# armlabstanford/Touch-GS

Measured on AMD Instinct MI355X. Metric: train iters/s (whole-job views/s) + render Mpix/s, 1M Gaussians @ 1080p, higher is better.
Workload: dtype f32; 1 GPU; configs[2]: 1M Gaussians, 1080p, full Touch-GS train loop (RGB L1/SSIM + tactile depth/uncertainty loss), one view per rank per iter; gaussians=1000000, width=1920, height=1080, sh_degree=3, views=8, tiles=8160, longest_tile_list_any_view=792, max_list_hint=1022, parallelism=dp1, layout=morton (model.spatial_sort(): same scene, rows permuted), depth_loss_type=DEPTH_UNCERTAINTY_WEIGHTED_LOSS

## Files before the change

### touch_gs_amd/csrc/imgloss.hip

```cpp
#include <math.h>
#include <stdlib.h>
#include "tgs_common.h"

namespace {

constexpr int WIN = 11, HALO = 5;
struct Win { float g[WIN]; };
#ifdef TGS_SSIM_SGPR_WINDOW
#define WK(k) win.g[k]
#else
__device__ constexpr float WGT[WIN] = {0x1.0d956cp-10f, 0x1.f1fe02p-8f, 0x1.26eb18p-5f, 0x1.bff0fep-4f, 0x1.b43c4p-3f,
                                       0x1.10656p-2f, 0x1.b43c4p-3f, 0x1.bff0fep-4f, 0x1.26eb18p-5f, 0x1.f1fe02p-8f,
                                       0x1.0d956cp-10f};
#define WK(k) WGT[k]
#endif

#ifndef TGS_SSIM_DMA
#define TGS_SSIM_DMA 0
#endif
constexpr int SW = 64;
constexpr int NTH = 3 * SW;
constexpr int RB = WIN;
__host__ __device__ constexpr int seg_rows(int nblk) { return RB * nblk - 2 * HALO; }

template <int CH>
struct RowBlock {
  static constexpr int ROWF = (SW + 2 * HALO) * CH;
  static constexpr int NIT = (RB * ROWF + NTH - 1) / NTH;
  template <int B = 8>
  static __device__ __forceinline__ void stage(const float* __restrict__ src, float* __restrict__ lds,
                                               int W, int H, int x0, int r0, int tid) {
#pragma unroll 1
    for (int it0 = 0; it0 < NIT; it0 += B) {
      float v[B];
#pragma unroll
      for (int u = 0; u < B; u++) {
        const int i = tid + NTH * (it0 + u);
        const int j = i / ROWF, e = i - j * ROWF;
        const int gy = r0 + j, gxf = (x0 - HALO) * CH + e;
        v[u] = 0.f;
        if (i < RB * ROWF && gy >= 0 && gy < H && gxf >= 0 && gxf < W * CH) v[u] = src[(size_t)gy * W * CH + gxf];
      }
#pragma unroll
      for (int u = 0; u < B; u++) {
        const int i = tid + NTH * (it0 + u);
        if (i < RB * ROWF) lds[i] = v[u];
      }
    }
  }
  static constexpr int PADF = (RB * ROWF + TGS_WAVE - 1) / TGS_WAVE * TGS_WAVE;
  static constexpr int NDMA = PADF / TGS_WAVE;
  static __device__ __forceinline__ void dma(__amdgpu_buffer_rsrc_t rsrc, float* __restrict__ lds, int W, int H, int x0, int r0, int tid) {
    typedef __attribute__((address_space(3))) float lds_float;
    const int wave = __builtin_amdgcn_readfirstlane(tid >> 6), lane = tid & 63;
    constexpr int NW = NTH / TGS_WAVE;
    const int gx0 = (x0 - HALO) * CH, WC = W * CH;
#pragma unroll
    for (int u = 0; u * NW < NDMA; u++) {
      const int chunk = u * NW + wave;
      if (chunk < NDMA) {
        const int i = chunk * TGS_WAVE + lane;
        const int j = i / ROWF, e = i - j * ROWF;
        const int gy = r0 + j, gxf = gx0 + e;
        const bool in = i < RB * ROWF && (unsigned)gy < (unsigned)H && (unsigned)gxf < (unsigned)WC;
        const unsigned off = in ? (unsigned)(gy * WC + gxf) * 4u : 0xffffffffu;
        __builtin_amdgcn_raw_ptr_buffer_load_lds(rsrc, (lds_float*)(lds + chunk * TGS_WAVE), 4, off, 0, 0, 0);
      }
    }
  }
  static __device__ __forceinline__ void stage2(const float* __restrict__ src_a, const float* __restrict__ src_b,
                                                float* __restrict__ lds_a, float* __restrict__ lds_b,
                                                int W, int H, int x0, int r0, int tid) {
#ifndef TGS_SSIM_FWD_B
#define TGS_SSIM_FWD_B 13
#endif
    constexpr int B = TGS_SSIM_FWD_B;
#pragma unroll 1
    for (int it0 = 0; it0 < NIT; it0 += B) {
      float va[B], vb[B];
#pragma unroll
      for (int u = 0; u < B; u++) {
        const int i = tid + NTH * (it0 + u);
        const int j = i / ROWF, e = i - j * ROWF;
        const int gy = r0 + j, gxf = (x0 - HALO) * CH + e;
        va[u] = 0.f; vb[u] = 0.f;
        if (it0 + u < NIT && i < RB * ROWF && gy >= 0 && gy < H && gxf >= 0 && gxf < W * CH) {
          const size_t o = (size_t)gy * W * CH + gxf;
          va[u] = src_a[o]; vb[u] = src_b[o];
        }
      }
#pragma unroll
      for (int u = 0; u < B; u++) {
        const int i = tid + NTH * (it0 + u);
        if (it0 + u < NIT && i < RB * ROWF) { lds_a[i] = va[u]; lds_b[i] = vb[u]; }
      }
    }
  }
};

__global__ __launch_bounds__(NTH) __attribute__((amdgpu_waves_per_eu(4, 8))) void k_ssim_fwd(int W, int H, Win win,
                                                  const float* __restrict__ img,
                                                  const float* __restrict__ gt,
                                                  float* __restrict__ adj ,
                                                  float* __restrict__ block_partials, int n_partials, int NBLK,
                                                  int y_lo, int y_hi, int c_lo, int c_hi) {
  const int SEG = seg_rows(NBLK);
  constexpr int ROWF = RowBlock<3>::ROWF;
#if TGS_SSIM_DMA & 1
  __shared__ float sa2[2][RowBlock<3>::PADF], sb2[2][RowBlock<3>::PADF];
  const __amdgpu_buffer_rsrc_t rs_a = __builtin_amdgcn_make_buffer_rsrc((void*)img, 0, (int)((size_t)W * H * 12), 0x00020000);
  const __amdgpu_buffer_rsrc_t rs_b = __builtin_amdgcn_make_buffer_rsrc((void*)gt, 0, (int)((size_t)W * H * 12), 0x00020000);
#else
  __shared__ float sa[RB * ROWF], sb[RB * ROWF];
#endif
  __shared__ float red[NTH / TGS_WAVE];
  const int tid = threadIdx.x;
  const int x0 = blockIdx.x * SW, ys = y_lo + blockIdx.y * SEG;
  const int gx = x0 + tid / 3, c = tid - (tid / 3) * 3;
  const int ye = min(ys + SEG, y_hi);
  float w[RB][5];
#pragma unroll
  for (int p = 0; p < RB; p++)
#pragma unroll
    for (int q = 0; q < 5; q++) w[p][q] = 0.f;
  float msum = 0.f;
#if TGS_SSIM_DMA & 1
  RowBlock<3>::dma(rs_a, sa2[0], W, H, x0, ys - HALO, tid);
  RowBlock<3>::dma(rs_b, sb2[0], W, H, x0, ys - HALO, tid);
#endif
  for (int blk = 0; blk < NBLK; blk++) {
    const int r0 = ys - HALO + blk * RB;
    if (r0 - HALO >= ye) break;
#if TGS_SSIM_DMA & 1
    asm volatile("s_waitcnt vmcnt(0)" ::: "memory");
    __syncthreads();
    if (blk + 1 < NBLK && r0 + RB - HALO < ye) {
      RowBlock<3>::dma(rs_a, sa2[(blk + 1) & 1], W, H, x0, r0 + RB, tid);
      RowBlock<3>::dma(rs_b, sb2[(blk + 1) & 1], W, H, x0, r0 + RB, tid);
    }
    const float* sa = sa2[blk & 1];
    const float* sb = sb2[blk & 1];
#else
    __syncthreads();
    {
      RowBlock<3>::stage2(img, gt, sa, sb, W, H, x0, r0, tid);
    }
    __syncthreads();
#endif
#pragma unroll
    for (int p = 0; p < RB; p++) {
      const float* ra = sa + p * ROWF + tid;
      const float* rb = sb + p * ROWF + tid;
      float m1 = 0.f, m2 = 0.f, e11 = 0.f, e22 = 0.f, e12 = 0.f;
#pragma unroll
      for (int k = 0; k < WIN; k++) {
        const float a = ra[3 * k], b = rb[3 * k];
        const float ga = WK(k) * a, gb = WK(k) * b;
        m1 += ga; m2 += gb;
        e11 = fmaf(ga, a, e11); e22 = fmaf(gb, b, e22); e12 = fmaf(ga, b, e12);
      }
      w[p][0] = m1; w[p][1] = m2; w[p][2] = e11; w[p][3] = e22; w[p][4] = e12;
      const int gy = r0 + p - HALO;
      if (gy >= ys && gy < ye) {
        float o[5] = {0.f, 0.f, 0.f, 0.f, 0.f};
#pragma unroll
        for (int k = 0; k < WIN; k++) {
#pragma unroll
          for (int q = 0; q < 5; q++) o[q] = fmaf(WK(k), w[(p + 1 + k) % RB][q], o[q]);
        }
        const float C1 = 0.01f * 0.01f, C2 = 0.03f * 0.03f;
        const float mu1 = o[0], mu2 = o[1];
        const float s11 = o[2] - mu1 * mu1, s22 = o[3] - mu2 * mu2, s12 = o[4] - mu1 * mu2;
        const float n1 = 2.f * mu1 * mu2 + C1, n2 = 2.f * s12 + C2;
        const float d1 = mu1 * mu1 + mu2 * mu2 + C1, d2 = s11 + s22 + C2;
        const float id1 = __builtin_amdgcn_rcpf(d1), id2 = __builtin_amdgcn_rcpf(d2);
        const float m = n1 * n2 * id1 * id2;
        if (gx < W) {
          if (gy >= c_lo && gy < c_hi) msum += m;
          if (adj) {
            const float dm_ds12 = 2.f * n1 * id1 * id2;
            const float dm_ds11 = -m * id2;
            const float dm_dmu1 = 2.f * mu2 * n2 * id1 * id2 - m * 2.f * mu1 * id1;
            float* o3 = adj + (((size_t)gy * W + gx) * 3 + c) * 3;
            o3[0] = dm_dmu1 - 2.f * mu1 * dm_ds11 - mu2 * dm_ds12;
            o3[1] = dm_ds11;
            o3[2] = dm_ds12;
          }
        }
      }
    }
  }
  const float tot = wave_sum(msum);
  if ((tid & 63) == 0) red[tid >> 6] = tot;
  __syncthreads();
  const int wg = blockIdx.y * gridDim.x + blockIdx.x, nwg = gridDim.x * gridDim.y;
  if (tid == 0) block_partials[wg] = red[0] + red[1] + red[2];
  for (int i = nwg + wg * NTH + tid; i < n_partials; i += nwg * NTH) block_partials[i] = 0.f;
}

__global__ __launch_bounds__(NTH) __attribute__((amdgpu_waves_per_eu(4, 8))) void k_ssim_bwd(int W, int H, Win win, float weight,
                                                  const float* __restrict__ img,
                                                  const float* __restrict__ gt,
                                                  const float* __restrict__ adj,
                                                  float* __restrict__ v_img, int NBLK, int y_lo, int y_hi) {
  const int SEG = seg_rows(NBLK);
  constexpr int ROWF = RowBlock<9>::ROWF;
#if TGS_SSIM_DMA & 2
  __shared__ float sadj2[2][RowBlock<9>::PADF];
  const __amdgpu_buffer_rsrc_t rs_j = __builtin_amdgcn_make_buffer_rsrc((void*)adj, 0, (int)((size_t)W * H * 36), 0x00020000);
#else
  __shared__ float sadj[RB * ROWF];
#endif
  const int tid = threadIdx.x;
  const int x0 = blockIdx.x * SW, ys = y_lo + blockIdx.y * SEG;
  const int gx = x0 + tid / 3;
  const int ye = min(ys + SEG, y_hi);
  float w[RB][3];
#pragma unroll
  for (int p = 0; p < RB; p++) { w[p][0] = 0.f; w[p][1] = 0.f; w[p][2] = 0.f; }
#if TGS_SSIM_DMA & 2
  RowBlock<9>::dma(rs_j, sadj2[0], W, H, x0, ys - HALO, tid);
#endif
  for (int blk = 0; blk < NBLK; blk++) {
    const int r0 = ys - HALO + blk * RB;
    if (r0 - HALO >= ye) break;
#if TGS_SSIM_DMA & 2
    asm volatile("s_waitcnt vmcnt(0)" ::: "memory");
    __syncthreads();
    if (blk + 1 < NBLK && r0 + RB - HALO < ye) RowBlock<9>::dma(rs_j, sadj2[(blk + 1) & 1], W, H, x0, r0 + RB, tid);
    const float* sadj = sadj2[blk & 1];
#else
    __syncthreads();
    {
#ifndef TGS_SSIM_BWD_B
#define TGS_SSIM_BWD_B 20
#endif
      RowBlock<9>::stage<TGS_SSIM_BWD_B>(adj, sadj, W, H, x0, r0, tid);
    }
    __syncthreads();
#endif
#pragma unroll
    for (int p = 0; p < RB; p++) {
      const float* r = sadj + p * ROWF + 3 * tid;
      float h0 = 0.f, h1 = 0.f, h2 = 0.f;
#pragma unroll
      for (int k = 0; k < WIN; k++) {
        h0 = fmaf(WK(k), r[9 * k], h0);
        h1 = fmaf(WK(k), r[9 * k + 1], h1);
        h2 = fmaf(WK(k), r[9 * k + 2], h2);
      }
      w[p][0] = h0; w[p][1] = h1; w[p][2] = h2;
      const int gy = r0 + p - HALO;
      if (gy >= ys && gy < ye) {
        float o0 = 0.f, o1 = 0.f, o2 = 0.f;
#pragma unroll
        for (int k = 0; k < WIN; k++) {
          o0 = fmaf(WK(k), w[(p + 1 + k) % RB][0], o0);
          o1 = fmaf(WK(k), w[(p + 1 + k) % RB][1], o1);
          o2 = fmaf(WK(k), w[(p + 1 + k) % RB][2], o2);
        }
        if (gx < W) {
          const size_t pidx = (size_t)gy * W * 3 + (size_t)x0 * 3 + tid;
          v_img[pidx] = weight * (o0 + 2.f * img[pidx] * o1 + gt[pidx] * o2);
        }
      }
    }
  }
}


constexpr int SWO = SW - 2 * HALO;
__host__ __device__ constexpr int fused_seg_rows(int nblk) { return RB * nblk - 4 * HALO; }

__global__ __launch_bounds__(NTH) __attribute__((amdgpu_waves_per_eu(3, 4))) void k_ssim_fused(
    int W, int H, float weight, const float* __restrict__ img, const float* __restrict__ gt,
    float* __restrict__ v_img, float* __restrict__ block_partials, int n_partials, int NBLK,
    int y_lo, int y_hi, int c_lo, int c_hi) {
  const int SEG = fused_seg_rows(NBLK);
  constexpr int ROWF = RowBlock<3>::ROWF;
  constexpr int ADJF = SW * 9;
  __shared__ float sa[RB * ROWF], sb[RB * ROWF];
  __shared__ float sadj[RB * ADJF];
  __shared__ float red[NTH / TGS_WAVE];
  const int tid = threadIdx.x;
  const int col = tid / 3, c = tid - col * 3;
  const int xa0 = blockIdx.x * SWO - HALO;
  const int gx = xa0 + col;
  const int ys = y_lo + blockIdx.y * SEG, ye = min(ys + SEG, y_hi);
  const bool own_col = col >= HALO && col < SW - HALO;
  const int cb = min(max(col - HALO, 0), SWO - 1);
  float w[RB][5], w2[RB][3];
#pragma unroll
  for (int p = 0; p < RB; p++) {
#pragma unroll
    for (int q = 0; q < 5; q++) w[p][q] = 0.f;
    w2[p][0] = 0.f; w2[p][1] = 0.f; w2[p][2] = 0.f;
  }
  float msum = 0.f;
  for (int blk = 0; blk < NBLK; blk++) {
    const int r0 = ys - 2 * HALO + blk * RB;
    if (r0 - 2 * HALO >= ye) break;
    __syncthreads();
    RowBlock<3>::stage2(img, gt, sa, sb, W, H, xa0, r0, tid);
    __syncthreads();
#pragma unroll
    for (int p = 0; p < RB; p++) {
      const float* ra = sa + p * ROWF + tid;
      const float* rb = sb + p * ROWF + tid;
      float m1 = 0.f, m2 = 0.f, e11 = 0.f, e22 = 0.f, e12 = 0.f;
#pragma unroll
      for (int k = 0; k < WIN; k++) {
        const float a = ra[3 * k], b = rb[3 * k];
        const float ga = WK(k) * a, gb = WK(k) * b;
        m1 += ga; m2 += gb;
        e11 = fmaf(ga, a, e11); e22 = fmaf(gb, b, e22); e12 = fmaf(ga, b, e12);
      }
      w[p][0] = m1; w[p][1] = m2; w[p][2] = e11; w[p][3] = e22; w[p][4] = e12;
      const int gy = r0 + p - HALO;
      float A = 0.f, B = 0.f, C = 0.f;
      if (gy >= ys - HALO && gy < ye + HALO && gy >= 0 && gy < H) {
        float o[5] = {0.f, 0.f, 0.f, 0.f, 0.f};
#pragma unroll
        for (int k = 0; k < WIN; k++) {
#pragma unroll
          for (int q = 0; q < 5; q++) o[q] = fmaf(WK(k), w[(p + 1 + k) % RB][q], o[q]);
        }
        const float C1 = 0.01f * 0.01f, C2 = 0.03f * 0.03f;
        const float mu1 = o[0], mu2 = o[1];
        const float s11 = o[2] - mu1 * mu1, s22 = o[3] - mu2 * mu2, s12 = o[4] - mu1 * mu2;
        const float n1 = 2.f * mu1 * mu2 + C1, n2 = 2.f * s12 + C2;
        const float d1 = mu1 * mu1 + mu2 * mu2 + C1, d2 = s11 + s22 + C2;
        const float id1 = __builtin_amdgcn_rcpf(d1), id2 = __builtin_amdgcn_rcpf(d2);
        const float m = n1 * n2 * id1 * id2;
        if (gx >= 0 && gx < W) {
          if (own_col && gy >= ys && gy < ye && gy >= c_lo && gy < c_hi) msum += m;
          const float dm_ds12 = 2.f * n1 * id1 * id2;
          const float dm_ds11 = -m * id2;
          const float dm_dmu1 = 2.f * mu2 * n2 * id1 * id2 - m * 2.f * mu1 * id1;
          A = dm_dmu1 - 2.f * mu1 * dm_ds11 - mu2 * dm_ds12;
          B = dm_ds11;
          C = dm_ds12;
        }
      }
      float* o3 = sadj + p * ADJF + tid * 3;
      o3[0] = A; o3[1] = B; o3[2] = C;
    }
    __syncthreads();
#pragma unroll
    for (int p = 0; p < RB; p++) {
      const float* r = sadj + p * ADJF + (cb * 3 + c) * 3;
      float h0 = 0.f, h1 = 0.f, h2 = 0.f;
#pragma unroll
      for (int k = 0; k < WIN; k++) {
        h0 = fmaf(WK(k), r[9 * k], h0);
        h1 = fmaf(WK(k), r[9 * k + 1], h1);
        h2 = fmaf(WK(k), r[9 * k + 2], h2);
      }
      w2[p][0] = h0; w2[p][1] = h1; w2[p][2] = h2;
      const int gy = r0 + p - 2 * HALO;
      if (gy >= ys && gy < ye) {
        float o0 = 0.f, o1 = 0.f, o2 = 0.f;
#pragma unroll
        for (int k = 0; k < WIN; k++) {
          o0 = fmaf(WK(k), w2[(p + 1 + k) % RB][0], o0);
          o1 = fmaf(WK(k), w2[(p + 1 + k) % RB][1], o1);
          o2 = fmaf(WK(k), w2[(p + 1 + k) % RB][2], o2);
        }
        if (own_col && gx < W) {
          const size_t pidx = ((size_t)gy * W + gx) * 3 + c;
          v_img[pidx] = weight * (o0 + 2.f * img[pidx] * o1 + gt[pidx] * o2);
        }
      }
    }
  }
  const float tot = wave_sum(msum);
  if ((tid & 63) == 0) red[tid >> 6] = tot;
  __syncthreads();
  const int wg = blockIdx.y * gridDim.x + blockIdx.x, nwg = gridDim.x * gridDim.y;
  if (tid == 0) block_partials[wg] = red[0] + red[1] + red[2];
  for (int i = nwg + wg * NTH + tid; i < n_partials; i += nwg * NTH) block_partials[i] = 0.f;
}

__global__ void k_ssim_zero_partials(float* __restrict__ block_partials, int n_partials) {
  const int i = blockIdx.x * blockDim.x + threadIdx.x;
  if (i < n_partials) block_partials[i] = 0.f;
}

}

static inline bool count_inside(int y0, int y1, int c0, int c1) { return c0 >= c1 || (c0 >= y0 && c1 <= y1); }

static int ssim_impl(int W, int H, const float* img, const float* gt, float weight,
                     float* block_partials, int n_partials, float* v_img, float* scratch,
                     int y0, int y1, int c0, int c1, void* stream) {
  TGS_CHECK_ARG(W > 0 && H > 0, "bad image size");
  TGS_CHECK_ARG(img && gt && block_partials, "null pointer");
  TGS_CHECK_ARG(!v_img || scratch, "gradient needs scratch");
  TGS_CHECK_ARG(0 <= y0 && y0 <= y1 && y1 <= H && y0 <= c0 && c0 <= c1 && c1 <= y1, "bad row range");
  Win win;
  double g[WIN], sum = 0.0;
  for (int i = 0; i < WIN; i++) { g[i] = exp(-(double)((i - HALO) * (i - HALO)) / (2.0 * 1.5 * 1.5)); sum += g[i]; }
  for (int i = 0; i < WIN; i++) win.g[i] = (float)(g[i] / sum);
  static const int env_nblk = [] { const char* e = getenv("TGS_SSIM_NBLK"); return e ? max(2, min(16, atoi(e))) : 0; }();
  static const int env_fused = [] { const char* e = getenv("TGS_SSIM_FUSED"); return e ? atoi(e) : 0; }();
  if (v_img && env_fused && y1 > y0 && count_inside(y0, y1, c0, c1)) {
    const int fx = (W + SWO - 1) / SWO;
    auto wgs = [&](int nb) { return (long long)fx * ((y1 - y0 + fused_seg_rows(nb) - 1) / fused_seg_rows(nb)); };
    int nblk = 7;
    while (nblk > 3 && wgs(nblk) < 600) nblk--;
    if (env_nblk) nblk = max(3, env_nblk);
    while (nblk < 16 && wgs(nblk) > n_partials) nblk++;
    TGS_CHECK_ARG(wgs(nblk) <= n_partials, "block_partials too small");
    const int SEGF = fused_seg_rows(nblk);
    hipLaunchKernelGGL(k_ssim_fused, dim3(fx, (y1 - y0 + SEGF - 1) / SEGF, 1), dim3(NTH), 0, (hipStream_t)stream, W, H, weight,
                       img, gt, v_img, block_partials, n_partials, nblk, y0, y1, c0, c1);
    TGS_CHECK_LAUNCH();
    return TGS_OK;
  }
  const int f0 = v_img ? max(0, y0 - HALO) : y0, f1 = v_img ? min(H, y1 + HALO) : y1;
  const int rows = f1 - f0;
  if (rows <= 0) {
    if (n_partials > 0) {
      hipLaunchKernelGGL(k_ssim_zero_partials, dim3((n_partials + 255) / 256), dim3(256), 0, (hipStream_t)stream, block_partials,
                         n_partials);
      TGS_CHECK_LAUNCH();
    }
    return TGS_OK;
  }
  const int sx = (W + SW - 1) / SW;
  int nblk = 4;
  while (nblk > 2 && (long long)sx * ((rows + seg_rows(nblk) - 1) / seg_rows(nblk)) < 3 * 256) nblk--;
  if (env_nblk) nblk = env_nblk;
  while (nblk < 16 && (long long)sx * ((rows + seg_rows(nblk) - 1) / seg_rows(nblk)) > n_partials) nblk++;
  TGS_CHECK_ARG((long long)sx * ((rows + seg_rows(nblk) - 1) / seg_rows(nblk)) <= n_partials, "block_partials too small");
  const int SEG = seg_rows(nblk);
  const dim3 block(NTH);
  hipStream_t s = (hipStream_t)stream;
  hipLaunchKernelGGL(k_ssim_fwd, dim3(sx, (rows + SEG - 1) / SEG, 1), block, 0, s, W, H, win, img, gt,
                     v_img ? scratch : nullptr, block_partials, n_partials, nblk, f0, f1, c0, c1);
  TGS_CHECK_LAUNCH();
  if (v_img && y1 > y0) {
    hipLaunchKernelGGL(k_ssim_bwd, dim3(sx, (y1 - y0 + SEG - 1) / SEG, 1), block, 0, s, W, H, win, weight, img, gt,
                       scratch, v_img, nblk, y0, y1);
    TGS_CHECK_LAUNCH();
  }
  return TGS_OK;
}

extern "C" int tgs_ssim_fwd_bwd(int W, int H, const float* img, const float* gt, float weight,
                                float* block_partials, float* v_img, float* scratch,
                                void* stream) {
  return ssim_impl(W, H, img, gt, weight, block_partials, ((W + 15) / 16) * ((H + 15) / 16), v_img, scratch,
                   0, H, 0, H, stream);
}

extern "C" int tgs_ssim_fwd_bwd_rows(int W, int H, const float* img, const float* gt, float weight,
                                     float* block_partials, int n_partials, float* v_img,
                                     float* scratch, int y0, int y1, int count_y0, int count_y1,
                                     void* stream) {
  return ssim_impl(W, H, img, gt, weight, block_partials, n_partials, v_img, scratch, y0, y1, count_y0,
                   count_y1, stream);
}
```

Baseline: 990.3 iters/s.

## Use buffer loads with precomputed offsets and occupancy-sized SSIM row segments

SSIM forward and backward staging now uses raw buffer loads. A per-thread offset map is computed once and advanced by a fixed stride per row block, and out-of-range elements rely on buffer bounds checking to return zero, replacing per-element index math and branches. Segment height is now chosen arbitrarily between two and four row blocks, sized from the device's resident workgroup count via an occupancy query, and the kernels exit early past the segment end. This aims to cut address and bounds overhead and to balance the grid against CU occupancy. It adds a host-side occupancy query and relies on buffer out-of-bounds semantics for correctness.

Result: slower. 977.6 iters/s (-1.3%).

```diff
diff --git a/touch_gs_amd/csrc/imgloss.hip b/touch_gs_amd/csrc/imgloss.hip
--- a/touch_gs_amd/csrc/imgloss.hip
+++ b/touch_gs_amd/csrc/imgloss.hip
@@ -1,5 +1,6 @@
 #include <math.h>
 #include <stdlib.h>
+#include <atomic>
 #include "tgs_common.h"
 
 namespace {
@@ -22,30 +23,49 @@
 constexpr int NTH = 3 * SW;
 constexpr int RB = WIN;
 __host__ __device__ constexpr int seg_rows(int nblk) { return RB * nblk - 2 * HALO; }
+__host__ __device__ constexpr int seg_blocks(int seg) { return (seg + 2 * HALO + RB - 1) / RB; }
+constexpr int SEG_MIN = seg_rows(2), SEG_MAX = seg_rows(4);
 
 template <int CH>
 struct RowBlock {
   static constexpr int ROWF = (SW + 2 * HALO) * CH;
   static constexpr int NIT = (RB * ROWF + NTH - 1) / NTH;
-  template <int B = 8>
-  static __device__ __forceinline__ void stage(const float* __restrict__ src, float* __restrict__ lds,
-                                               int W, int H, int x0, int r0, int tid) {
-#pragma unroll 1
-    for (int it0 = 0; it0 < NIT; it0 += B) {
-      float v[B];
-#pragma unroll
-      for (int u = 0; u < B; u++) {
-        const int i = tid + NTH * (it0 + u);
-        const int j = i / ROWF, e = i - j * ROWF;
-        const int gy = r0 + j, gxf = (x0 - HALO) * CH + e;
-        v[u] = 0.f;
-        if (i < RB * ROWF && gy >= 0 && gy < H && gxf >= 0 && gxf < W * CH) v[u] = src[(size_t)gy * W * CH + gxf];
-      }
-#pragma unroll
-      for (int u = 0; u < B; u++) {
-        const int i = tid + NTH * (it0 + u);
-        if (i < RB * ROWF) lds[i] = v[u];
-      }
+  static constexpr int STAGEF = NIT * NTH;
+  static constexpr unsigned OOR = 0x80000000u;
+  struct Map { unsigned off[NIT]; };
+  static __device__ __forceinline__ void make_map(Map& m, int W, int x0, int rel, int tid) {
+#pragma unroll
+    for (int it = 0; it < NIT; it++) {
+      const int i = tid + NTH * it;
+      const int j = i / ROWF, e = i - j * ROWF;
+      const int gxf = (x0 - HALO) * CH + e;
+      m.off[it] = ((i < RB * ROWF && gxf >= 0 && gxf < W * CH) ? (unsigned)(j * W * CH + gxf) * 4u : OOR) + (unsigned)rel;
+    }
+  }
+  static constexpr int MAXW = 1 << 18;
+  static __device__ __forceinline__ __amdgpu_buffer_rsrc_t rows(const float* src, int W, int r_lo, int r_hi) {
+    return __builtin_amdgcn_make_buffer_rsrc((void*)(src + (size_t)r_lo * W * CH), 0, (r_hi - r_lo) * W * CH * 4, 0x00020000);
+  }
+  static __device__ __forceinline__ float load(__amdgpu_buffer_rsrc_t rs, unsigned off) {
+    return __builtin_bit_cast(float, __builtin_amdgcn_raw_buffer_load_b32(rs, (int)off, 0, 0));
+  }
+  static __device__ __forceinline__ void stage(__amdgpu_buffer_rsrc_t rs, float* __restrict__ lds, Map& m, int step, int tid) {
+    float v[NIT];
+#pragma unroll
+    for (int it = 0; it < NIT; it++) v[it] = load(rs, m.off[it]);
+#pragma unroll
+    for (int it = 0; it < NIT; it++) { lds[tid + NTH * it] = v[it]; m.off[it] += (unsigned)step; }
+  }
+  static __device__ __forceinline__ void stage_pair(__amdgpu_buffer_rsrc_t rs_a, __amdgpu_buffer_rsrc_t rs_b,
+                                                    float* __restrict__ lds_a, float* __restrict__ lds_b, Map& m, int step,
+                                                    int tid) {
+    float va[NIT], vb[NIT];
+#pragma unroll
+    for (int it = 0; it < NIT; it++) { va[it] = load(rs_a, m.off[it]); vb[it] = load(rs_b, m.off[it]); }
+#pragma unroll
+    for (int it = 0; it < NIT; it++) {
+      lds_a[tid + NTH * it] = va[it]; lds_b[tid + NTH * it] = vb[it];
+      m.off[it] += (unsigned)step;
     }
   }
   static constexpr int PADF = (RB * ROWF + TGS_WAVE - 1) / TGS_WAVE * TGS_WAVE;
@@ -102,16 +122,15 @@
                                                   const float* __restrict__ img,
                                                   const float* __restrict__ gt,
                                                   float* __restrict__ adj ,
-                                                  float* __restrict__ block_partials, int n_partials, int NBLK,
+                                                  float* __restrict__ block_partials, int n_partials, int NBLK, int SEG,
                                                   int y_lo, int y_hi, int c_lo, int c_hi) {
-  const int SEG = seg_rows(NBLK);
   constexpr int ROWF = RowBlock<3>::ROWF;
 #if TGS_SSIM_DMA & 1
   __shared__ float sa2[2][RowBlock<3>::PADF], sb2[2][RowBlock<3>::PADF];
   const __amdgpu_buffer_rsrc_t rs_a = __builtin_amdgcn_make_buffer_rsrc((void*)img, 0, (int)((size_t)W * H * 12), 0x00020000);
   const __amdgpu_buffer_rsrc_t rs_b = __builtin_amdgcn_make_buffer_rsrc((void*)gt, 0, (int)((size_t)W * H * 12), 0x00020000);
 #else
-  __shared__ float sa[RB * ROWF], sb[RB * ROWF];
+  __shared__ float sa[RowBlock<3>::STAGEF], sb[RowBlock<3>::STAGEF];
 #endif
   __shared__ float red[NTH / TGS_WAVE];
   const int tid = threadIdx.x;
@@ -127,6 +146,11 @@
 #if TGS_SSIM_DMA & 1
   RowBlock<3>::dma(rs_a, sa2[0], W, H, x0, ys - HALO, tid);
   RowBlock<3>::dma(rs_b, sb2[0], W, H, x0, ys - HALO, tid);
+#else
+  const int rlo = max(ys - HALO, 0), rhi = min(ye + HALO, H);
+  const __amdgpu_buffer_rsrc_t rs_a = RowBlock<3>::rows(img, W, rlo, rhi), rs_b = RowBlock<3>::rows(gt, W, rlo, rhi);
+  RowBlock<3>::Map map;
+  RowBlock<3>::make_map(map, W, x0, (ys - HALO - rlo) * W * 3 * 4, tid);
 #endif
   for (int blk = 0; blk < NBLK; blk++) {
     const int r0 = ys - HALO + blk * RB;
@@ -143,12 +167,13 @@
 #else
     __syncthreads();
     {
-      RowBlock<3>::stage2(img, gt, sa, sb, W, H, x0, r0, tid);
+      RowBlock<3>::stage_pair(rs_a, rs_b, sa, sb, map, RB * W * 3 * 4, tid);
     }
     __syncthreads();
 #endif
 #pragma unroll
     for (int p = 0; p < RB; p++) {
+      if (r0 + p >= ye + HALO) break;
       const float* ra = sa + p * ROWF + tid;
       const float* rb = sb + p * ROWF + tid;
       float m1 = 0.f, m2 = 0.f, e11 = 0.f, e22 = 0.f, e12 = 0.f;
@@ -202,14 +227,13 @@
                                                   const float* __restrict__ img,
                                                   const float* __restrict__ gt,
                                                   const float* __restrict__ adj,
-                                                  float* __restrict__ v_img, int NBLK, int y_lo, int y_hi) {
-  const int SEG = seg_rows(NBLK);
+                                                  float* __restrict__ v_img, int NBLK, int SEG, int y_lo, int y_hi) {
   constexpr int ROWF = RowBlock<9>::ROWF;
 #if TGS_SSIM_DMA & 2
   __shared__ float sadj2[2][RowBlock<9>::PADF];
   const __amdgpu_buffer_rsrc_t rs_j = __builtin_amdgcn_make_buffer_rsrc((void*)adj, 0, (int)((size_t)W * H * 36), 0x00020000);
 #else
-  __shared__ float sadj[RB * ROWF];
+  __shared__ float sadj[RowBlock<9>::STAGEF];
 #endif
   const int tid = threadIdx.x;
   const int x0 = blockIdx.x * SW, ys = y_lo + blockIdx.y * SEG;
@@ -220,6 +244,11 @@
   for (int p = 0; p < RB; p++) { w[p][0] = 0.f; w[p][1] = 0.f; w[p][2] = 0.f; }
 #if TGS_SSIM_DMA & 2
   RowBlock<9>::dma(rs_j, sadj2[0], W, H, x0, ys - HALO, tid);
+#else
+  const int rlo = max(ys - HALO, 0);
+  const __amdgpu_buffer_rsrc_t rs_j = RowBlock<9>::rows(adj, W, rlo, min(ye + HALO, H));
+  RowBlock<9>::Map map;
+  RowBlock<9>::make_map(map, W, x0, (ys - HALO - rlo) * W * 9 * 4, tid);
 #endif
   for (int blk = 0; blk < NBLK; blk++) {
     const int r0 = ys - HALO + blk * RB;
@@ -231,16 +260,12 @@
     const float* sadj = sadj2[blk & 1];
 #else
     __syncthreads();
-    {
-#ifndef TGS_SSIM_BWD_B
-#define TGS_SSIM_BWD_B 20
-#endif
-      RowBlock<9>::stage<TGS_SSIM_BWD_B>(adj, sadj, W, H, x0, r0, tid);
-    }
+    RowBlock<9>::stage(rs_j, sadj, map, RB * W * 9 * 4, tid);
     __syncthreads();
 #endif
 #pragma unroll
     for (int p = 0; p < RB; p++) {
+      if (r0 + p >= ye + HALO) break;
       const float* r = sadj + p * ROWF + 3 * tid;
       float h0 = 0.f, h1 = 0.f, h2 = 0.f;
 #pragma unroll
@@ -390,6 +415,24 @@
 
 static inline bool count_inside(int y0, int y1, int c0, int c1) { return c0 >= c1 || (c0 >= y0 && c1 <= y1); }
 
+static int ssim_resident_workgroups() {
+  constexpr int MAXDEV = 64;
+  static std::atomic<int> cache[MAXDEV];
+  int dev = 0;
+  if (hipGetDevice(&dev) != hipSuccess || dev < 0 || dev >= MAXDEV) return 0;
+  int v = cache[dev].load(std::memory_order_relaxed);
+  if (v == 0) {
+    int cus = 0, fwd = 0, bwd = 0;
+    if (hipDeviceGetAttribute(&cus, hipDeviceAttributeMultiprocessorCount, dev) != hipSuccess ||
+        hipOccupancyMaxActiveBlocksPerMultiprocessor(&fwd, k_ssim_fwd, NTH, 0) != hipSuccess ||
+        hipOccupancyMaxActiveBlocksPerMultiprocessor(&bwd, k_ssim_bwd, NTH, 0) != hipSuccess)
+      return 0;
+    v = cus * min(fwd, bwd);
+    cache[dev].store(v, std::memory_order_relaxed);
+  }
+  return v;
+}
+
 static int ssim_impl(int W, int H, const float* img, const float* gt, float weight,
                      float* block_partials, int n_partials, float* v_img, float* scratch,
                      int y0, int y1, int c0, int c1, void* stream) {
@@ -401,7 +444,8 @@
   double g[WIN], sum = 0.0;
   for (int i = 0; i < WIN; i++) { g[i] = exp(-(double)((i - HALO) * (i - HALO)) / (2.0 * 1.5 * 1.5)); sum += g[i]; }
   for (int i = 0; i < WIN; i++) win.g[i] = (float)(g[i] / sum);
-  static const int env_nblk = [] { const char* e = getenv("TGS_SSIM_NBLK"); return e ? max(2, min(16, atoi(e))) : 0; }();
+  const char* e_nblk = getenv("TGS_SSIM_NBLK");
+  const int env_nblk = e_nblk ? max(2, min(16, atoi(e_nblk))) : 0;
   static const int env_fused = [] { const char* e = getenv("TGS_SSIM_FUSED"); return e ? atoi(e) : 0; }();
   if (v_img && env_fused && y1 > y0 && count_inside(y0, y1, c0, c1)) {
     const int fx = (W + SWO - 1) / SWO;
@@ -427,21 +471,29 @@
     }
     return TGS_OK;
   }
+  TGS_CHECK_ARG(W <= RowBlock<9>::MAXW, "image too wide");
   const int sx = (W + SW - 1) / SW;
-  int nblk = 4;
-  while (nblk > 2 && (long long)sx * ((rows + seg_rows(nblk) - 1) / seg_rows(nblk)) < 3 * 256) nblk--;
-  if (env_nblk) nblk = env_nblk;
-  while (nblk < 16 && (long long)sx * ((rows + seg_rows(nblk) - 1) / seg_rows(nblk)) > n_partials) nblk++;
-  TGS_CHECK_ARG((long long)sx * ((rows + seg_rows(nblk) - 1) / seg_rows(nblk)) <= n_partials, "block_partials too small");
-  const int SEG = seg_rows(nblk);
+  const int slots = ssim_resident_workgroups();
+  TGS_CHECK_ARG(slots > 0, "occupancy query failed");
+  const int ny_max = max(1, slots / sx);
+  int SEG = min(SEG_MAX, max(SEG_MIN, (rows + ny_max - 1) / ny_max));
+  if (env_nblk) SEG = seg_rows(env_nblk);
+  auto wgs = [&](int seg) { return (long long)sx * ((rows + seg - 1) / seg); };
+  if (wgs(SEG) > n_partials) {
+    int nb = seg_blocks(SEG);
+    while (nb < 16 && wgs(seg_rows(nb)) > n_partials) nb++;
+    SEG = seg_rows(nb);
+  }
+  TGS_CHECK_ARG(wgs(SEG) <= n_partials, "block_partials too small");
+  const int nblk = seg_blocks(SEG);
   const dim3 block(NTH);
   hipStream_t s = (hipStream_t)stream;
   hipLaunchKernelGGL(k_ssim_fwd, dim3(sx, (rows + SEG - 1) / SEG, 1), block, 0, s, W, H, win, img, gt,
-                     v_img ? scratch : nullptr, block_partials, n_partials, nblk, f0, f1, c0, c1);
+                     v_img ? scratch : nullptr, block_partials, n_partials, nblk, SEG, f0, f1, c0, c1);
   TGS_CHECK_LAUNCH();
   if (v_img && y1 > y0) {
     hipLaunchKernelGGL(k_ssim_bwd, dim3(sx, (y1 - y0 + SEG - 1) / SEG, 1), block, 0, s, W, H, win, weight, img, gt,
-                       scratch, v_img, nblk, y0, y1);
+                       scratch, v_img, nblk, SEG, y0, y1);
     TGS_CHECK_LAUNCH();
   }
   return TGS_OK;
```

## Precompute SSIM row-block staging address plan and add optional register prefetch

Applied to the files above, without the earlier changes.

Replaces the per-element division and bounds checks in the SSIM LDS staging loops with a per-thread plan. The plan is computed once per block and holds column-validity bitmasks and byte offsets, and each row block only applies a cheap row mask. The staging loops are fully unrolled. An optional, default-off mode prefetches the next row block into registers while the current one is being computed. This adds register pressure and more complex addressing.

Measured after the change: 1019 iters/s before, 1022 iters/s after (median of 6 runs). About the same (+0.3%).

```diff
diff --git a/touch_gs_amd/csrc/imgloss.hip b/touch_gs_amd/csrc/imgloss.hip
--- a/touch_gs_amd/csrc/imgloss.hip
+++ b/touch_gs_amd/csrc/imgloss.hip
@@ -1,22 +1,26 @@
 #include <math.h>
 #include <stdlib.h>
+#include <type_traits>
 #include "tgs_common.h"
 
 namespace {
 
 constexpr int WIN = 11, HALO = 5;
 struct Win { float g[WIN]; };
-#ifdef TGS_SSIM_SGPR_WINDOW
-#define WK(k) win.g[k]
-#else
 __device__ constexpr float WGT[WIN] = {0x1.0d956cp-10f, 0x1.f1fe02p-8f, 0x1.26eb18p-5f, 0x1.bff0fep-4f, 0x1.b43c4p-3f,
                                        0x1.10656p-2f, 0x1.b43c4p-3f, 0x1.bff0fep-4f, 0x1.26eb18p-5f, 0x1.f1fe02p-8f,
                                        0x1.0d956cp-10f};
+#ifdef TGS_SSIM_SGPR_WINDOW
+#define WK(k) win.g[k]
+#else
 #define WK(k) WGT[k]
 #endif
 
 #ifndef TGS_SSIM_DMA
 #define TGS_SSIM_DMA 0
+#endif
+#ifndef TGS_SSIM_PREFETCH
+#define TGS_SSIM_PREFETCH 0
 #endif
 constexpr int SW = 64;
 constexpr int NTH = 3 * SW;
@@ -27,25 +31,103 @@
 struct RowBlock {
   static constexpr int ROWF = (SW + 2 * HALO) * CH;
   static constexpr int NIT = (RB * ROWF + NTH - 1) / NTH;
+  static_assert(NTH <= ROWF && NIT <= 64, "the plan keeps one bit per element and two candidate rows");
+  typedef typename std::conditional<(NIT <= 32), unsigned, unsigned long long>::type mask_t;
+  static constexpr int j_lo(int it) { return NTH * it / ROWF; }
+  static constexpr int tid_hi(int it) { return ROWF * (j_lo(it) + 1) - NTH * it; }
+  static constexpr mask_t its_of_row(int j, int d) {
+    mask_t m = 0;
+    for (int it = 0; it < NIT; it++)
+      if (j_lo(it) + d == j) m |= (mask_t)1 << it;
+    return m;
+  }
+  struct Plan {
+    mask_t lo, hi;
+    unsigned v_lo, v_hi;
+    unsigned pitch;
+    unsigned pad;
+  };
+  static __device__ __forceinline__ Plan plan(int W, int x0, int tid) {
+    Plan P;
+    P.pitch = (unsigned)W * (CH * 4);
+    P.pad = P.pitch < ROWF * 4u ? ROWF * 4u - P.pitch : 0u;
+    P.v_lo = 4u * tid + P.pad;
+    P.v_hi = P.v_lo + P.pitch - ROWF * 4u;
+    P.lo = 0; P.hi = 0;
+    const int gx0 = (x0 - HALO) * CH, WC = W * CH;
+#pragma unroll
+    for (int it = 0; it < NIT; it++) {
+      const int i = tid + NTH * it;
+      const bool up = tid >= tid_hi(it);
+      const int e = i - (j_lo(it) + (up ? 1 : 0)) * ROWF;
+      if (i < RB * ROWF && gx0 + e >= 0 && gx0 + e < WC) {
+        if (up) P.hi |= (mask_t)1 << it; else P.lo |= (mask_t)1 << it;
+      }
+    }
+    return P;
+  }
+  struct Block { mask_t in, hi; };
+  static __device__ __forceinline__ Block block(const Plan& P, int r0, int H) {
+    mask_t lo = 0, hi = 0;
+#pragma unroll
+    for (int j = 0; j < RB; j++)
+      if ((unsigned)(r0 + j) < (unsigned)H) { lo |= its_of_row(j, 0); hi |= its_of_row(j, 1); }
+    hi &= P.hi;
+    return Block{(P.lo & lo) | hi, hi};
+  }
+  static __device__ __forceinline__ const char* origin(const Plan& P, const float* __restrict__ src, int W, int x0, int r0) {
+    return (const char*)src + (((long long)r0 * W + (x0 - HALO)) * (CH * 4) - (long long)P.pad);
+  }
+  static __device__ __forceinline__ bool inside(const Block& K, int it) { return (K.in >> it) & 1; }
+  static __device__ __forceinline__ const float* addr(const Plan& P, const Block& K, const char* org, int it) {
+    const char* row = org + ((size_t)j_lo(it) * P.pitch + 4 * (NTH * it - j_lo(it) * ROWF));
+    const unsigned v = tid_hi(it) < NTH && ((K.hi >> it) & 1) ? P.v_hi : P.v_lo;
+    return (const float*)(row + v);
+  }
+  static __device__ __forceinline__ void put(float* __restrict__ lds, int tid, int it, float v) {
+    if (it < NIT - 1 || tid < RB * ROWF - NTH * (NIT - 1)) lds[tid + NTH * it] = v;
+  }
+  static __device__ __forceinline__ void fetch(const Plan& P, const float* __restrict__ src, int W, int H, int x0, int r0,
+                                               float (&v)[NIT]) {
+    const Block K = block(P, r0, H);
+    const char* org = origin(P, src, W, x0, r0);
+#pragma unroll
+    for (int it = 0; it < NIT; it++) {
+      v[it] = 0.f;
+      if (inside(K, it)) v[it] = *addr(P, K, org, it);
+    }
+  }
+  static __device__ __forceinline__ void store(float* __restrict__ lds, int tid, const float (&v)[NIT]) {
+#pragma unroll
+    for (int it = 0; it < NIT; it++) put(lds, tid, it, v[it]);
+  }
+  static __device__ __forceinline__ void fetch2(const Plan& P, const float* __restrict__ src_a, const float* __restrict__ src_b,
+                                                int W, int H, int x0, int r0, float (&va)[NIT], float (&vb)[NIT]) {
+    const Block K = block(P, r0, H);
+    const char* org_a = origin(P, src_a, W, x0, r0);
+    const char* org_b = origin(P, src_b, W, x0, r0);
+#pragma unroll
+    for (int it = 0; it < NIT; it++) {
+      va[it] = 0.f; vb[it] = 0.f;
+      if (inside(K, it)) { va[it] = *addr(P, K, org_a, it); vb[it] = *addr(P, K, org_b, it); }
+    }
+  }
   template <int B = 8>
-  static __device__ __forceinline__ void stage(const float* __restrict__ src, float* __restrict__ lds,
+  static __device__ __forceinline__ void stage(const Plan& P, const float* __restrict__ src, float* __restrict__ lds,
                                                int W, int H, int x0, int r0, int tid) {
-#pragma unroll 1
+    const Block K = block(P, r0, H);
+    const char* org = origin(P, src, W, x0, r0);
+#pragma unroll
     for (int it0 = 0; it0 < NIT; it0 += B) {
       float v[B];
 #pragma unroll
       for (int u = 0; u < B; u++) {
-        const int i = tid + NTH * (it0 + u);
-        const int j = i / ROWF, e = i - j * ROWF;
-        const int gy = r0 + j, gxf = (x0 - HALO) * CH + e;
         v[u] = 0.f;
-        if (i < RB * ROWF && gy >= 0 && gy < H && gxf >= 0 && gxf < W * CH) v[u] = src[(size_t)gy * W * CH + gxf];
-      }
-#pragma unroll
-      for (int u = 0; u < B; u++) {
-        const int i = tid + NTH * (it0 + u);
-        if (i < RB * ROWF) lds[i] = v[u];
-      }
+        if (it0 + u < NIT && inside(K, it0 + u)) v[u] = *addr(P, K, org, it0 + u);
+      }
+#pragma unroll
+      for (int u = 0; u < B; u++)
+        if (it0 + u < NIT) put(lds, tid, it0 + u, v[u]);
     }
   }
   static constexpr int PADF = (RB * ROWF + TGS_WAVE - 1) / TGS_WAVE * TGS_WAVE;
@@ -68,32 +150,27 @@
       }
     }
   }
-  static __device__ __forceinline__ void stage2(const float* __restrict__ src_a, const float* __restrict__ src_b,
+  static __device__ __forceinline__ void stage2(const Plan& P, const float* __restrict__ src_a, const float* __restrict__ src_b,
                                                 float* __restrict__ lds_a, float* __restrict__ lds_b,
                                                 int W, int H, int x0, int r0, int tid) {
 #ifndef TGS_SSIM_FWD_B
 #define TGS_SSIM_FWD_B 13
 #endif
     constexpr int B = TGS_SSIM_FWD_B;
-#pragma unroll 1
+    const Block K = block(P, r0, H);
+    const char* org_a = origin(P, src_a, W, x0, r0);
+    const char* org_b = origin(P, src_b, W, x0, r0);
+#pragma unroll
     for (int it0 = 0; it0 < NIT; it0 += B) {
       float va[B], vb[B];
 #pragma unroll
       for (int u = 0; u < B; u++) {
-        const int i = tid + NTH * (it0 + u);
-        const int j = i / ROWF, e = i - j * ROWF;
-        const int gy = r0 + j, gxf = (x0 - HALO) * CH + e;
         va[u] = 0.f; vb[u] = 0.f;
-        if (it0 + u < NIT && i < RB * ROWF && gy >= 0 && gy < H && gxf >= 0 && gxf < W * CH) {
-          const size_t o = (size_t)gy * W * CH + gxf;
-          va[u] = src_a[o]; vb[u] = src_b[o];
-        }
-      }
-#pragma unroll
-      for (int u = 0; u < B; u++) {
-        const int i = tid + NTH * (it0 + u);
-        if (it0 + u < NIT && i < RB * ROWF) { lds_a[i] = va[u]; lds_b[i] = vb[u]; }
-      }
+        if (it0 + u < NIT && inside(K, it0 + u)) { va[u] = *addr(P, K, org_a, it0 + u); vb[u] = *addr(P, K, org_b, it0 + u); }
+      }
+#pragma unroll
+      for (int u = 0; u < B; u++)
+        if (it0 + u < NIT) { put(lds_a, tid, it0 + u, va[u]); put(lds_b, tid, it0 + u, vb[u]); }
     }
   }
 };
@@ -127,6 +204,14 @@
 #if TGS_SSIM_DMA & 1
   RowBlock<3>::dma(rs_a, sa2[0], W, H, x0, ys - HALO, tid);
   RowBlock<3>::dma(rs_b, sb2[0], W, H, x0, ys - HALO, tid);
+#else
+  constexpr bool PREFETCH = TGS_SSIM_PREFETCH & 1;
+  const RowBlock<3>::Plan plan = RowBlock<3>::plan(W, x0, tid);
+  float na[RowBlock<3>::NIT], nb[RowBlock<3>::NIT];
+  if (PREFETCH) {
+    RowBlock<3>::stage2(plan, img, gt, sa, sb, W, H, x0, ys - HALO, tid);
+    __syncthreads();
+  }
 #endif
   for (int blk = 0; blk < NBLK; blk++) {
     const int r0 = ys - HALO + blk * RB;
@@ -141,11 +226,13 @@
     const float* sa = sa2[blk & 1];
     const float* sb = sb2[blk & 1];
 #else
-    __syncthreads();
-    {
-      RowBlock<3>::stage2(img, gt, sa, sb, W, H, x0, r0, tid);
-    }
-    __syncthreads();
+    if (!PREFETCH) {
+      __syncthreads();
+      RowBlock<3>::stage2(plan, img, gt, sa, sb, W, H, x0, r0, tid);
+      __syncthreads();
+    }
+    const bool more = PREFETCH && blk + 1 < NBLK && r0 + RB - HALO < ye;
+    if (more) RowBlock<3>::fetch2(plan, img, gt, W, H, x0, r0 + RB, na, nb);
 #endif
 #pragma unroll
     for (int p = 0; p < RB; p++) {
@@ -189,6 +276,14 @@
         }
       }
     }
+#if !(TGS_SSIM_DMA & 1)
+    if (more) {
+      __syncthreads();
+      RowBlock<3>::store(sa, tid, na);
+      RowBlock<3>::store(sb, tid, nb);
+      __syncthreads();
+    }
+#endif
   }
   const float tot = wave_sum(msum);
   if ((tid & 63) == 0) red[tid >> 6] = tot;
@@ -198,6 +293,9 @@
   for (int i = nwg + wg * NTH + tid; i < n_partials; i += nwg * NTH) block_partials[i] = 0.f;
 }
 
+#ifndef TGS_SSIM_BWD_B
+#define TGS_SSIM_BWD_B 20
+#endif
 __global__ __launch_bounds__(NTH) __attribute__((amdgpu_waves_per_eu(4, 8))) void k_ssim_bwd(int W, int H, Win win, float weight,
                                                   const float* __restrict__ img,
                                                   const float* __restrict__ gt,
@@ -220,6 +318,14 @@
   for (int p = 0; p < RB; p++) { w[p][0] = 0.f; w[p][1] = 0.f; w[p][2] = 0.f; }
 #if TGS_SSIM_DMA & 2
   RowBlock<9>::dma(rs_j, sadj2[0], W, H, x0, ys - HALO, tid);
+#else
+  constexpr bool PREFETCH = (TGS_SSIM_PREFETCH & 2) != 0;
+  const RowBlock<9>::Plan plan = RowBlock<9>::plan(W, x0, tid);
+  float nj[RowBlock<9>::NIT];
+  if (PREFETCH) {
+    RowBlock<9>::stage<TGS_SSIM_BWD_B>(plan, adj, sadj, W, H, x0, ys - HALO, tid);
+    __syncthreads();
+  }
 #endif
   for (int blk = 0; blk < NBLK; blk++) {
     const int r0 = ys - HALO + blk * RB;
@@ -230,14 +336,13 @@
     if (blk + 1 < NBLK && r0 + RB - HALO < ye) RowBlock<9>::dma(rs_j, sadj2[(blk + 1) & 1], W, H, x0, r0 + RB, tid);
     const float* sadj = sadj2[blk & 1];
 #else
-    __syncthreads();
-    {
-#ifndef TGS_SSIM_BWD_B
-#define TGS_SSIM_BWD_B 20
-#endif
-      RowBlock<9>::stage<TGS_SSIM_BWD_B>(adj, sadj, W, H, x0, r0, tid);
-    }
-    __syncthreads();
+    if (!PREFETCH) {
+      __syncthreads();
+      RowBlock<9>::stage<TGS_SSIM_BWD_B>(plan, adj, sadj, W, H, x0, r0, tid);
+      __syncthreads();
+    }
+    const bool more = PREFETCH && blk + 1 < NBLK && r0 + RB - HALO < ye;
+    if (more) RowBlock<9>::fetch(plan, adj, W, H, x0, r0 + RB, nj);
 #endif
 #pragma unroll
     for (int p = 0; p < RB; p++) {
@@ -265,6 +370,13 @@
         }
       }
     }
+#if !(TGS_SSIM_DMA & 2)
+    if (more) {
+      __syncthreads();
+      RowBlock<9>::store(sadj, tid, nj);
+      __syncthreads();
+    }
+#endif
   }
 }
 
@@ -277,6 +389,9 @@
     float* __restrict__ v_img, float* __restrict__ block_partials, int n_partials, int NBLK,
     int y_lo, int y_hi, int c_lo, int c_hi) {
   const int SEG = fused_seg_rows(NBLK);
+#ifdef TGS_SSIM_SGPR_WINDOW
+  constexpr Win win = {{WGT[0], WGT[1], WGT[2], WGT[3], WGT[4], WGT[5], WGT[6], WGT[7], WGT[8], WGT[9], WGT[10]}};
+#endif
   constexpr int ROWF = RowBlock<3>::ROWF;
   constexpr int ADJF = SW * 9;
   __shared__ float sa[RB * ROWF], sb[RB * ROWF];
@@ -297,11 +412,12 @@
     w2[p][0] = 0.f; w2[p][1] = 0.f; w2[p][2] = 0.f;
   }
   float msum = 0.f;
+  const RowBlock<3>::Plan plan = RowBlock<3>::plan(W, xa0, tid);
   for (int blk = 0; blk < NBLK; blk++) {
     const int r0 = ys - 2 * HALO + blk * RB;
     if (r0 - 2 * HALO >= ye) break;
     __syncthreads();
-    RowBlock<3>::stage2(img, gt, sa, sb, W, H, xa0, r0, tid);
+    RowBlock<3>::stage2(plan, img, gt, sa, sb, W, H, xa0, r0, tid);
     __syncthreads();
 #pragma unroll
     for (int p = 0; p < RB; p++) {
```
